# uber/aresdb

Hardware: AMD Instinct MI355X
Metric: rows/sec, 1B-row filter -> group-by-agg (whole job) (higher is better)
Workload: dtype u32 keys / f64 sums; 1 GPU; C3: filter d1<90 -> dims [floor(ts,3600), d1, d2, d3] (4 x uint32) -> SUM(m float32 -> float64) via HashReduce, validity bitmaps with 1% nulls, shard resident in HBM; rows_per_gpu=1000000000, batch_rows=67108864, batches=15, streams_per_query=2, parallelism=1 shard(s), one per GPU

## Files before the change

aresdb_amd/csrc/algo/hr_rtc_gen.hip:

```cpp
#include <cstdio>
#include <functional>
#include <sstream>
#include <string>
#include <vector>

#include "hr_kernels.hpp"
#include "hr_rtc_gen.hpp"

namespace ares {

namespace {

bool int_kind(int k) { return k == K_I32 || k == K_U32; }
bool col_kind(int k) { return k == K_I32 || k == K_U32 || k == K_F32; }

std::string hex(uint32_t v) {
  char b[16];
  snprintf(b, sizeof(b), "0x%08xu", v);
  return b;
}

std::string const_name(int slot) { return "a.k[" + std::to_string(slot) + "]"; }

bool gen_value(const RtcExpr &f, std::ostringstream &o, const char *v, const char *okb, const char *r, const std::string &kc,
// ... 692 lines not shown
         "  i0 = i0c;\n";
    for (int c = 0; c < nc; c++) {
      if (nullMask & (1u << c)) o << "  okc[" << c << "] = (r.win[" << c << "] >> ((i0c + a.bitOff[" << c << "]) & 7u)) & 0xFu;\n";
      else o << "  okc[" << c << "] = 0xFu;\n";
    }
    o << "#pragma unroll\n"
         "  for (int j = 0; j < 4; j++) {\n"
         "    u32 keep = ((u32)j >= sh && (int)(i0c + j) < a.length) ? 1u : 0u;\n";
    for (int k = 0; k < s.numFilters; k++) {
      const RtcExpr &e = s.filters[k];
      if (e.col < 0 || e.col >= nc) return "";
      o << "    {\n      const u32 v = r.v[" << e.col << "][j]; const u32 okb = (okc[" << e.col << "] >> j) & 1u;\n";
      if (!gen_compare(e, o, "v", "okb", "keep", const_name(const_slot_filter(k)))) return "";
      o << "    }\n";
    }
    o << "    alive[j] = keep;\n  }\n";
    for (int c = firstFilterCol; c < nc; c++) prefetch(c);
    if (constMeasure) {
      o << "  cv[0] = cv[1] = cv[2] = cv[3] = " << const_name(const_slot_measure()) << ";\n";
    } else {
      const RtcExpr &e = s.measure;
      if (e.col != nd) return "";
      o << "#pragma unroll\n  for (int j = 0; j < 4; j++) {\n"
           "    const u32 v = r.v[" << nd << "][j]; const u32 okb = (okc[" << nd << "] >> j) & 1u; u32 x;\n";
      if (!gen_value(e, o, "v", "okb", "x", const_name(const_slot_measure()), sort64)) return "";
      if (avg) {
        const int rk = e.rk;
        if (!(rk == K_F32 || rk == K_I32 || rk == K_U32) || !(s.measureDtype == Float64 || s.measureDtype == Int64)) return "";
        const bool f64 = s.measureDtype == Float64;
        const char *cvt = rk == K_F32 ? (f64 ? "x" : "__float_as_uint((float)(i64)__uint_as_float(x))")
                          : rk == K_I32 ? (f64 ? "__float_as_uint((float)(double)(i32)x)" : "__float_as_uint((float)(i64)(i32)x)")
                                        : (f64 ? "__float_as_uint((float)(double)x)" : "__float_as_uint((float)(i64)x)");
        o << "    cv[j] = okb ? " << cvt << " : 0u;\n"
             "    alive[j] |= (alive[j] & (okb ^ 1u)) << 31;\n";
      } else if (s.measureWidth == 8) {
        if (s.identity != 0) return "";
        o << "    cv[j] = okb ? x : 0u;\n";
      } else {
        const int target = s.measureDtype == Int32 ? K_I32 : s.measureDtype == Uint32 ? K_U32 : K_F32;
        if (!plain_store(e.rk, target)) return "";
        o << "    cv[j] = okb ? x : " << hex(static_cast<uint32_t>(s.identity)) << ";\n";
      }
      o << "  }\n";
      prefetch(nd);
    }
    if (SL.all4 && !sort64) {
    o << "  u32 h[4] = {0u, 0u, 0u, 0u}, okbytes[4] = {0u, 0u, 0u, 0u};\n";
    for (int d = 0; d < nd; d++) {
      const RtcExpr &e = s.dims[d];
      if (e.col != d || !plain_store(e.rk, e.outKind)) return "";
      o << "#pragma unroll\n  for (int j = 0; j < 4; j++) {\n"
           "    const u32 v = r.v[" << d << "][j]; const u32 okb = (okc[" << d << "] >> j) & 1u; u32 x;\n";
      if (!gen_value(e, o, "v", "okb", "x", const_name(const_slot_dim(d)))) return "";
      o << "    h[j] = mix(h[j], x); okbytes[j] |= okb << " << 8 * d << ";\n  }\n";
      prefetch(d);
    }
    o << "#pragma unroll\n  for (int j = 0; j < 4; j++) {\n    u32 g = h[j];\n";
    if (nd == 4) o << "    g = mix(g, okbytes[j]);\n";
    else o << "    { u32 k = okbytes[j] * 0xcc9e2d51u; k = rotl(k, 15) * 0x1b873593u; g ^= k; }\n";
    o << "    g ^= " << 5 * nd << "u; g ^= g >> 16; g *= 0x85ebca6bu; g ^= g >> 13; g *= 0xc2b2ae35u; g ^= g >> 16;\n"
         "    hh[j] = g;\n  }\n}\n";
    } else {
      for (int d = 0; d < nd; d++) o << "  u32 xv" << d << "[4], xo" << d << "[4];\n";
      for (int d = 0; d < nd; d++) {
        const RtcExpr &e = s.dims[d];
        if (e.col != d || !plain_store(e.rk, e.outKind) || (SL.width[d] != 4 && !int_kind(e.rk))) return "";
        o << "#pragma unroll\n  for (int j = 0; j < 4; j++) {\n"
             "    const u32 v = r.v[" << d << "][j]; const u32 okb = (okc[" << d << "] >> j) & 1u; u32 x;\n";
        if (!gen_value(e, o, "v", "okb", "x", const_name(const_slot_dim(d)))) return "";
        o << "    xv" << d << "[j] = x" << width_mask(SL.width[d]) << "; xo" << d << "[j] = okb;\n  }\n";
        prefetch(d);
      }
      o << "#pragma unroll\n  for (int j = 0; j < 4; j++) {\n";
      if (sort64) {
        o << "    u64 h64;\n";
        gen_row_hash64(o, SL, [](int d, int) { return "xv" + std::to_string(d) + "[j]"; }, [](int d) { return "xo" + std::to_string(d) + "[j]"; },
                       "h64", "    ");
        o << "    hh[j] = (u32)(h64 >> 32); cw[j] = (u32)h64;\n";
      } else {
        gen_row_hash(o, SL, [](int d) { return "xv" + std::to_string(d) + "[j]"; }, [](int d) { return "xo" + std::to_string(d) + "[j]"; },
                     "hh[j]", "    ");
      }
      o << "  }\n}\n";
    }
  }
  if (kind == RTC_SCAN_TABLE) {
    if (!gen_widen(o, s) || !gen_agg(o, s)) return "";
    kernel_body_table(o);
  } else if (kind == RTC_SCAN_COMPACT) {
    kernel_body_compact(o, s);
  } else {
    Lines16 rec{sort64 ? "cw[j]" : "0u"};
    if (avg) rec.row = "(a.rowBase + i0 + j) | (alive[j] & 0x80000000u)";
    kernel_body_lines16(o, s, rec);
  }
  return o.str();
}

std::string generate_vector(const RtcSpec &s) {
  const int nd = s.nd, vw = s.vectorVW, partBits = s.partBits;
  const bool hll = s.kind == RTC_HLL_SCAN, sort64 = hll || s.kind == RTC_SORT_VECTOR_SCAN;
  if (nd < 1 || nd > (sort64 ? kFusedDims : kGenericFusedDims) || (vw != 4 && vw != 8) || (sort64 && vw != 4)) return "";
  if (hll && (partBits < 1 || partBits > 9)) return "";
  const SlotLayout SL = slot_layout(s.dimWidth, nd, sort64 ? 16 : 4);
  if (!SL.ok || (!sort64 && !SL.all4)) return "";
  const int *width = SL.width;
  int wb[kFusedDims] = {};
  bool narrow = false, wide = false;
  int nw = 0;
  for (int d = 0; d < nd; d++) {
    narrow = narrow || width[d] != 4;
    wide = wide || width[d] > 4;
    wb[d] = nw;
    nw += width[d] > 4 ? width[d] / 4 : 1;
  }
  if (wide && SL.valueBytes > kSortVectorValueBytes) return "";
  std::ostringstream o;
  const int mq = vw / 4;
  o << kPrelude << (sort64 ? kPrelude64 : "") << args_text()
    << "#define ND " << nd << "\n#define MQ " << mq << "\n#define PB " << partBits << "\n#define NP " << (1 << partBits) << "\n";
  if (wide) o << "#define NW " << nw << "\nstruct Raw { u32 v[NW][4]; u32 ok[ND]; u32 m[MQ * 4]; };\n";
  else o << "struct Raw { u32 v[ND][4]; u32 ok[ND]; u32 m[MQ * 4]; };\n";
  o << "__device__ __forceinline__ void load_full(Raw &r, const Args &a, u32 i0) {\n";
  if (narrow) {
    for (int d = 0; d < nd; d++) {
      const int v = wb[d];
      if (width[d] > 4) {
        const int q = width[d] / 4;
        o << "  {\n    const PU32x4 *p = reinterpret_cast<const PU32x4 *>(reinterpret_cast<const u8 *>(a.vals[" << d << "]) + " << width[d] << "ull * i0);\n";
        for (int k = 0; k < q; k++) o << "    const PU32x4 t" << k << " = p[" << k << "];\n";
        o << "   ";
        for (int k = 0; k < q; k++)
          for (int e = 0; e < 4; e++) o << " r.v[" << v + (4 * k + e) % q << "][" << (4 * k + e) / q << "] = t" << k << ".v[" << e << "];";
        o << "\n  }\n";
      } else if (width[d] == 4)
        o << "  { const PU32x4 t = *reinterpret_cast<const PU32x4 *>(a.vals[" << d << "] + i0); r.v[" << v << "][0] = t.v[0]; r.v[" << v
          << "][1] = t.v[1]; r.v[" << v << "][2] = t.v[2]; r.v[" << v << "][3] = t.v[3]; }\n";
      else if (width[d] == 2)
        o << "  { const PU32x2 t = *reinterpret_cast<const PU32x2 *>(reinterpret_cast<const u8 *>(a.vals[" << d << "]) + 2ull * i0); r.v[" << v
          << "][0] = t.v[0] & 0xFFFFu; r.v[" << v << "][1] = t.v[0] >> 16; r.v[" << v << "][2] = t.v[1] & 0xFFFFu; r.v[" << v << "][3] = t.v[1] >> 16; }\n";
      else
        o << "  { const u32 t = reinterpret_cast<const PU32 *>(reinterpret_cast<const u8 *>(a.vals[" << d << "]) + i0)->v; r.v[" << v
          << "][0] = t & 0xFFu; r.v[" << v << "][1] = (t >> 8) & 0xFFu; r.v[" << v << "][2] = (t >> 16) & 0xFFu; r.v[" << v << "][3] = t >> 24; }\n";
      o << "  r.ok[" << d << "] = reinterpret_cast<const PU32 *>(a.nulls[" << d << "] + i0)->v;\n";
    }
  } else {
  o << "#pragma unroll\n"
       "  for (int d = 0; d < ND; d++) {\n"
       "    const PU32x4 t = *reinterpret_cast<const PU32x4 *>(a.vals[d] + i0);\n"
       "    r.v[d][0] = t.v[0]; r.v[d][1] = t.v[1]; r.v[d][2] = t.v[2]; r.v[d][3] = t.v[3];\n"
       "    r.ok[d] = reinterpret_cast<const PU32 *>(a.nulls[d] + i0)->v;\n"
       "  }\n";
  }
  o << ""
       "#pragma unroll\n"
       "  for (int q = 0; q < MQ; q++) {\n"
       "    const PU32x4 t = *reinterpret_cast<const PU32x4 *>(a.vals[ND] + (u64)i0 * MQ + 4 * q);\n"
       "    r.m[4 * q] = t.v[0]; r.m[4 * q + 1] = t.v[1]; r.m[4 * q + 2] = t.v[2]; r.m[4 * q + 3] = t.v[3];\n"
       "  }\n"
       "}\n"
       "__device__ __forceinline__ void load_tail(Raw &r, const Args &a, u32 i0) {\n";
  if (narrow) {
    for (int d = 0; d < nd; d++) {
      const char *elem = width[d] == 4 ? "a.vals[%d][i0 + j]" : width[d] == 2 ? "(u32)reinterpret_cast<const u16 *>(a.vals[%d])[i0 + j]" : "(u32)reinterpret_cast<const u8 *>(a.vals[%d])[i0 + j]";
      char buf[128];
      snprintf(buf, sizeof(buf), elem, d);
      o << "  r.ok[" << d << "] = 0u;\n"
           "  for (int j = 0; j < 4; j++) {\n"
           "    const bool in = (int)(i0 + j) < a.length;\n";
      if (width[d] > 4)
        for (int k = 0; k < width[d] / 4; k++)
          o << "    r.v[" << wb[d] + k << "][j] = in ? a.vals[" << d << "][" << width[d] / 4 << "ull * (i0 + j) + " << k << "] : 0u;\n";
      else
        o << "    r.v[" << wb[d] << "][j] = in ? " << buf << " : 0u;\n";
      o << "    r.ok[" << d << "] |= in ? (u32)a.nulls[" << d << "][i0 + j] << (8 * j) : 0u;\n"
           "  }\n";
    }
  } else {
  o << "#pragma unroll\n"
       "  for (int d = 0; d < ND; d++) {\n"
       "    r.ok[d] = 0u;\n"
       "    for (int j = 0; j < 4; j++) {\n"
       "      const bool in = (int)(i0 + j) < a.length;\n"
       "      r.v[d][j] = in ? a.vals[d][i0 + j] : 0u;\n"
       "      r.ok[d] |= in ? (u32)a.nulls[d][i0 + j] << (8 * j) : 0u;\n"
       "    }\n"
       "  }\n";
  }
  o << "  for (int j = 0; j < 4; j++)\n"
       "    for (int q = 0; q < MQ; q++) r.m[j * MQ + q] = (int)(i0 + j) < a.length ? a.vals[ND][(u64)(i0 + j) * MQ + q] : 0u;\n"
       "}\n"
       "__device__ __forceinline__ void eval4(const Raw &r, const Args &a, u32 i0, u32 (&hh)[4], u32 (&cv)[4], u32 (&cw)[4], u32 (&alive)[4]) {\n"
       "#pragma unroll\n"
       "  for (int j = 0; j < 4; j++) {\n"
       "    alive[j] = (int)(i0 + j) < a.length ? 1u : 0u;\n";
  if (sort64) {
    o << "    u64 h64;\n";
    gen_row_hash64(o, SL, [&](int d, int k) { return "r.v[" + std::to_string(wb[d] + k) + "][j]"; },
                   [](int d) { return "((r.ok[" + std::to_string(d) + "] >> (8 * j)) & 0xFFu)"; }, "h64", "    ");
    if (hll) o << "    h64 = (h64 & 0xFFFFFFFFFFFF0000ull) | (u64)(r.m[j] & 0x3FFFu);\n";
    o << "    hh[j] = (u32)(h64 >> 32);\n"
         "    cv[j] = r.m[j];\n"
         "    cw[j] = (u32)h64;\n"
         "  }\n"
         "}\n";
  } else {
  o << "    u32 h = 0u, okbytes = 0u;\n"
       "#pragma unroll\n"
       "    for (int d = 0; d < ND; d++) { h = mix(h, r.v[d][j]); okbytes |= ((r.ok[d] >> (8 * j)) & 0xFFu) << (8 * d); }\n";
  if (nd == 4) o << "    h = mix(h, okbytes);\n";
  else o << "    { u32 k = okbytes * 0xcc9e2d51u; k = rotl(k, 15) * 0x1b873593u; h ^= k; }\n";
  o << "    h ^= " << 5 * nd << "u; h ^= h >> 16; h *= 0x85ebca6bu; h ^= h >> 13; h *= 0xc2b2ae35u; h ^= h >> 16;\n"
       "    hh[j] = h;\n"
       "    cv[j] = r.m[j * MQ];\n"
       "    cw[j] = MQ == 2 ? r.m[j * MQ + MQ - 1] : 0u;\n"
       "  }\n"
       "}\n";
  }
  o << "__device__ __forceinline__ void load_tile(Raw &r, const Args &a, u32 i0) { if ((int)(i0 + 3u) < a.length) load_full(r, a, i0); else if ((int)i0 < a.length) load_tail(r, a, i0); }\n"
       "__device__ __forceinline__ void eval4p(Raw &r, const Args &a, u32 &i0, u32 (&hh)[4], u32 (&cv)[4], u32 (&cw)[4], u32 (&alive)[4], u32 i0n) {\n"
       "  eval4(r, a, i0, hh, cv, cw, alive);\n"
       "  load_tile(r, a, i0n);\n"
       "}\n";
  Lines16 rec{"cw[j]"};
  if (hll)
    rec.part = "(((hh[j] ^ (cw[j] * 0x9E3779B1u)) * 0x85EBCA6Bu) >> (32 - PB))";
  else if (sort64)
    rec.part = "(a.pad ? (((hh[j] >> a.chunkTiles) ^ ((((hh[j] >> a.chunkTiles) >> PB) * 0x9E3779B1u) >> 23)) & (NP - 1u)) "
               ": (PB ? hh[j] >> (32 - (PB ? PB : 1)) : 0u))";
  kernel_body_lines16(o, s, rec);
  return o.str();
}

std::string generate_merge(const RtcSpec &s) {
  const int nd = s.nd, partBits = s.partBits, image = s.image, vectorVW = s.kind == RTC_VECTOR_MERGE ? s.vectorVW : 0;
  const bool compact = s.compact != 0, regionA = s.regionA != 0;
  if (nd < 1 || nd > kFusedDims) return "";
  if (image && vectorVW) return "";
  if (compact && (vectorVW || partBits < 3)) return "";
  if (partBits < 2) return "";
  const SlotLayout SL = slot_layout(s.dimWidth, nd, 4);
  if (!SL.ok || (vectorVW && !SL.all4)) return "";
  std::ostringstream o;
  o << kPrelude
    << "struct MArgs { const u32 *vals[" << kFusedCols << "]; const u8 *nulls[" << kFusedCols << "]; const u32 *recB; const u32 *countsB;\n"
       "  const u32 *prevRanges; const u8 *prevDims; const u8 *prevValues; u8 *dimOut; u8 *outValues; u32 *outCount; u32 *outRanges;\n"
       "  u64 prevCapacity, outCapacity; u32 bitOff[" << kFusedCols << "]; u32 capB, streams, prevSize, chunkRows; u64 *phases; u32 k[" << kNumConsts << "]; u32 pad;\n"
       "  const uint4 *recA; const u32 *cursorsA; u64 capA;\n"
       "  const uint4 *imgIn; uint4 *imgOut; const u32 *imgInCount; u32 *imgOutCount; u32 *hostOut; u32 knownOut, pad2; };\n"
       "#define FINISH() { __syncthreads(); if (threadIdx.x == 0u && a.hostOut) { __threadfence(); \\\n"
       "  if (atomicAdd(a.outCount + 4, 1u) == gridDim.x - 1u) { __threadfence(); const volatile u32 *oc = a.outCount; \\\n"
       "    a.hostOut[0] = oc[0]; a.hostOut[1] = oc[1]; a.hostOut[2] = oc[2]; a.hostOut[3] = oc[3]; } } }\n"
       "#define ND " << nd << "\n#define VB " << SL.valueBytes << "\n#define PB " << partBits << "\n#define NP " << (1 << partBits) << "\n"
       "#define SLOTS " << hr::kSlots << "\n#define LIMIT " << hr::kMergeLimit << "u\n#define RANGEWORDS " << hr::kRangeWords
    << "\n#define MAXRANGES " << hr::kMaxRanges << "u\n"
       "#define HMASK ((1u << (32 - PB)) - 1u)\n#define OCC 0x40000000u\n#define NEWG 0x80000000u\n";
  gen_widen(o, s);
  if (!gen_agg(o, s)) return "";
  if (s.phases)
    o << "#define STAMP(k) if (threadIdx.x == 0u) a.phases[(u64)blockIdx.x * 8u + (k)] = __builtin_amdgcn_s_memrealtime();\n";
  else
    o << "#define STAMP(k)\n";
  o << "#define BUCKETS (SLOTS / 4)\n"
       "struct Probe { u32 b, slot; bool done, isNew; };\n"
       "__device__ __forceinline__ void probe_round(u32 *sKeys, u32 *sClaimed, u32 *sOverflow, Probe &q, u32 want, u32 claimKey) {\n"
       "  const uint4 k = *reinterpret_cast<const uint4 *>(sKeys + 4u * q.b);\n"
       "  const bool e0 = k.x == 0u, e1 = k.y == 0u, e2 = k.z == 0u, e3 = k.w == 0u;\n"
       "  const bool m0 = (k.x & ~NEWG) == want, m1 = (k.y & ~NEWG) == want, m2 = (k.z & ~NEWG) == want, m3 = (k.w & ~NEWG) == want;\n"
       "  const bool anyM = m0 | m1 | m2 | m3, anyE = e0 | e1 | e2 | e3;\n"
       "  const u32 mi = m0 ? 0u : m1 ? 1u : m2 ? 2u : 3u, ei = e0 ? 0u : e1 ? 1u : e2 ? 2u : 3u;\n"
       "  const u32 mk = m0 ? k.x : m1 ? k.y : m2 ? k.z : k.w;\n"
       "  const bool active = !q.done, hit = active & anyM;\n"
       "  q.slot = hit ? 4u * q.b + mi : q.slot;\n"
       "  q.isNew = hit ? (mk & NEWG) != 0u : q.isNew;\n"
       "  bool claimed = false;\n"
       "  if (active & !anyM & anyE) {\n"
       "    u32 expected = 0u;\n"
       "    if (__hip_atomic_compare_exchange_strong(sKeys + 4u * q.b + ei, &expected, claimKey, __ATOMIC_RELAXED, __ATOMIC_RELAXED, __HIP_MEMORY_SCOPE_WORKGROUP)) {\n"
       "      if (__hip_atomic_fetch_add(sClaimed, 1u, __ATOMIC_RELAXED, __HIP_MEMORY_SCOPE_WORKGROUP) >= LIMIT)\n"
       "        __hip_atomic_store(sOverflow, 1u, __ATOMIC_RELAXED, __HIP_MEMORY_SCOPE_WORKGROUP);\n"
       "      q.slot = 4u * q.b + ei; q.isNew = true; claimed = true;\n"
       "    }\n"
       "  }\n"
       "  q.b = (active & !anyM & !anyE) ? (q.b + 1u) & (BUCKETS - 1u) : q.b;\n"
       "  q.done = q.done | hit | claimed;\n"
       "}\n"
       "__device__ __forceinline__ void insert(u32 *sKeys, u32 *sRows, u64 *sVals, u32 *sClaimed, u32 *sOverflow, u32 row, u32 h, u64 value, bool batch) {\n"
       "  const u32 want = (h & HMASK) | OCC;\n"
       "  Probe q; q.b = h & (BUCKETS - 1u); q.slot = 0u; q.done = false; q.isNew = false;\n"
       "  for (u32 tries = 0u; tries < 4u * BUCKETS && !q.done; tries++) probe_round(sKeys, sClaimed, sOverflow, q, want, batch ? want | NEWG : want);\n"
       "  if (q.done) {\n"
       "    if (q.isNew || !batch) __hip_atomic_fetch_min(sRows + q.slot, row, __ATOMIC_RELAXED, __HIP_MEMORY_SCOPE_WORKGROUP);\n"
       "    agg(sVals + q.slot, value);\n"
       "  } else {\n"
       "    __hip_atomic_store(sOverflow, 1u, __ATOMIC_RELAXED, __HIP_MEMORY_SCOPE_WORKGROUP);\n"
       "  }\n"
       "}\n";
  if (vectorVW == 8)
    o << "#define QCAP 96u\n#define QW 4u\n#define QDRAIN 32u\n#define VALB(z, w) ((((u64)(w)) << 32) | (z))\n";
  else if (vectorVW == 4)
    o << "#define QCAP 128u\n#define QW 3u\n#define QDRAIN 64u\n#define VALB(z, w) ((u64)(z))\n";
  else
    o << "#define QCAP 128u\n#define QW 3u\n#define QDRAIN 64u\n#define VALB(z, w) widen(z)\n";
  o << "struct Seg { const uint4 *ptr; u32 n, rem, rb; };\n"
       "struct Stage { uint4 r[4]; u32 n[4], rem[4], rb[4]; };\n"
       "__device__ __forceinline__ void drain(u32 *queue, u32 first, u32 count, u32 lane, u32 *sKeys, u32 *sRows, u64 *sVals, u32 *sClaimed, u32 *sOverflow) {\n"
       "  asm volatile(\"s_waitcnt lgkmcnt(0)\" ::: \"memory\");\n"
       "  if (lane < count) {\n"
       "    const u32 e = QW * (first + lane);\n"
       "    const u32 row = queue[e], h = queue[e + 1u], z = queue[e + 2u], w = QW == 4u ? queue[e + QW - 1u] : 0u;\n"
       "    insert(sKeys, sRows, sVals, sClaimed, sOverflow, row, h, VALB(z, w), true);\n"
       "  }\n"
       "  asm volatile(\"s_waitcnt lgkmcnt(0)\" ::: \"memory\");\n"
       "}\n"
       "__device__ __forceinline__ void consume_one(bool valid, u32 row, u32 h, u32 z, u32 w, u32 lane, u32 *sKeys, u32 *sRows, u64 *sVals, u32 *sClaimed, u32 *sOverflow, u32 *queue, u32 &qn) {\n"
       "  const u32 b = h & (BUCKETS - 1u), want = (h & HMASK) | OCC;\n"
       "  const uint4 k = *reinterpret_cast<const uint4 *>(sKeys + 4u * b);\n"
       "  const bool m0 = (k.x & ~NEWG) == want, m1 = (k.y & ~NEWG) == want, m2 = (k.z & ~NEWG) == want, m3 = (k.w & ~NEWG) == want;\n"
       "  const bool hit = valid && (m0 || m1 || m2 || m3);\n"
       "  if (hit) {\n"
       "    const u32 mi = m0 ? 0u : m1 ? 1u : m2 ? 2u : 3u;\n"
       "    const u32 mk = m0 ? k.x : m1 ? k.y : m2 ? k.z : k.w;\n"
       "    if (mk & NEWG) __hip_atomic_fetch_min(sRows + 4u * b + mi, row, __ATOMIC_RELAXED, __HIP_MEMORY_SCOPE_WORKGROUP);\n"
       "    agg(sVals + 4u * b + mi, VALB(z, w));\n"
       "  }\n"
       "  const bool pend = valid && !hit;\n"
       "  const u64 m = __ballot(pend);\n"
       "  if (m) {\n"
       "    if (pend) {\n"
       "      const u32 e = QW * (qn + __builtin_amdgcn_mbcnt_hi((u32)(m >> 32), __builtin_amdgcn_mbcnt_lo((u32)m, 0u)));\n"
       "      queue[e] = row; queue[e + 1u] = h; queue[e + 2u] = z;\n"
       "      if (QW == 4u) queue[e + QW - 1u] = w;\n"
       "    }\n"
       "    qn += (u32)__popcll(m);\n"
       "    if (qn >= QDRAIN) { const u32 take = qn < 64u ? qn : 64u; qn -= take; drain(queue, qn, take, lane, sKeys, sRows, sVals, sClaimed, sOverflow); }\n"
       "  }\n"
       "}\n";
  if (compact)
    o << "__device__ __forceinline__ void consume(const Stage &s, u32 lane, u32 p, u32 *sKeys, u32 *sRows, u64 *sVals, u32 *sClaimed, u32 *sOverflow, u32 *queue, u32 &qn) {\n"
         "  const u32 pos = 2u * (lane & 3u);\n"
         "  const u32 recBase = (lane >> 3) * 14u + 7u * ((lane >> 2) & 1u);\n"
         "#pragma unroll\n"
         "  for (int k = 0; k < 4; k++) {\n"
         "    const u64 hdr = ((u64)(u32)__builtin_amdgcn_mov_dpp((int)s.r[k].y, 0x00, 0xF, 0xF, true) << 32) | (u32)__builtin_amdgcn_mov_dpp((int)s.r[k].x, 0x00, 0xF, 0xF, true);\n"
         "#pragma unroll\n"
         "    for (u32 j = 0u; j < 2u; j++) {\n"
         "      const u32 ph = pos + j;\n"
         "      const u32 k7 = ph ? ph - 1u : 0u;\n"
         "      const bool valid = lane < s.n[k] && ph != 0u && recBase + k7 < s.rem[k];\n"
         "      const u32 z = j ? s.r[k].z : s.r[k].x, hw = j ? s.r[k].w : s.r[k].y;\n"
         "      const u32 lo9 = (u32)(hdr >> (9u * k7)) & 511u;\n"
         "      const u32 h = (p << (32 - PB)) | (hw >> PB);\n"
         "      const u32 row = s.rb[k] + (((hw & ((1u << PB) - 1u)) << 9) | lo9);\n"
         "      consume_one(valid, row, h, z, 0u, lane, sKeys, sRows, sVals, sClaimed, sOverflow, queue, qn);\n"
         "    }\n"
         "  }\n"
         "}\n";
  else
    o << "__device__ __forceinline__ void consume(const Stage &s, u32 lane, u32 p, u32 *sKeys, u32 *sRows, u64 *sVals, u32 *sClaimed, u32 *sOverflow, u32 *queue, u32 &qn) {\n"
         "#pragma unroll\n"
         "  for (int k = 0; k < 4; k++) {\n"
         "    const bool valid = lane < s.n[k] && s.r[k].x != 0xFFFFFFFFu;\n"
         "    consume_one(valid, s.r[k].x, s.r[k].y, s.r[k].z, s.r[k].w, lane, sKeys, sRows, sVals, sClaimed, sOverflow, queue, qn);\n"
         "  }\n"
         "}\n";
  if (!vectorVW) o << "__device__ __forceinline__ void eval_row(const MArgs &a, u32 row, u32 (&bits)[ND], u32 (&ok)[ND]) {\n";
  for (int d = 0; d < nd && !vectorVW; d++) {
    const RtcExpr &e = s.dims[d];
    const int c = e.col;
    if (c < 0 || c >= kFusedCols || !plain_store(e.rk, e.outKind) || (SL.width[d] != 4 && !int_kind(e.rk))) return "";
    o << "  {\n    const u32 v = " << column_elem(s.step[c], e.akind == K_I32, "a.vals[" + std::to_string(c) + "]", "row") << ";\n";
    if (s.nullMask & (1u << c)) o << "    const u32 bit = row + a.bitOff[" << c << "]; const u32 okb = (a.nulls[" << c << "][bit >> 3] >> (bit & 7u)) & 1u;\n";
    else o << "    const u32 okb = 1u;\n";
    o << "    u32 x;\n";
    if (!gen_value(e, o, "v", "okb", "x", const_name(const_slot_dim(d)))) return "";
    o << "    bits[" << d << "] = x; ok[" << d << "] = okb;\n  }\n";
  }
  if (!vectorVW) o << "}\n";
  const bool wide = s.aggWidth == 8;
  o << "extern \"C\" __global__ void __launch_bounds__(1024) hr_merge_rtc(MArgs a) {\n"
       "  __shared__ __attribute__((aligned(16))) u32 sKeys[SLOTS];\n"
       "  __shared__ __attribute__((aligned(16))) u32 sRows[SLOTS];\n"
       "  __shared__ __attribute__((aligned(16))) u64 sVals[SLOTS];\n"
       "  __shared__ u32 sRunCount[256];\n"
       "  __shared__ u32 sQueue[16u * QCAP * QW];\n"
       "  __shared__ u32 sClaimed, sOverflow, sCount, sBase, sEmit;\n"
       "  const u32 tid = threadIdx.x, lane = tid & 63u, wave = tid >> 6, p = blockIdx.x;\n"
       "  STAMP(0)\n";
  if (image == 2)
    o << "  {\n"
         "    const uint4 *img = a.imgIn + (u64)p * SLOTS;\n"
         "    for (u32 i = tid; i < SLOTS / 4u; i += 1024u) {\n"
         "      reinterpret_cast<uint4 *>(sKeys)[i] = img[i];\n"
         "      reinterpret_cast<uint4 *>(sRows)[i] = img[SLOTS / 4u + i];\n"
         "    }\n"
         "    for (u32 i = tid; i < SLOTS / 2u; i += 1024u) reinterpret_cast<uint4 *>(sVals)[i] = img[SLOTS / 2u + i];\n"
         "    if (tid == 0u) { sClaimed = a.imgInCount[p]; sOverflow = 0u; sCount = 0u; sEmit = 0u; }\n"
         "  }\n";
  else
    o << "  for (u32 s = tid; s < SLOTS; s += 1024u) { sKeys[s] = 0u; sRows[s] = 0xFFFFFFFFu; sVals[s] = IDENT; }\n"
         "  if (tid == 0u) { sClaimed = 0u; sOverflow = 0u; sCount = 0u; sEmit = 0u; }\n";
  o << "  const u32 G = a.streams;\n"
       "  if (tid < G) sRunCount[tid] = a.countsB[(u64)tid * NP + p];\n"
       "  const u32 *ranges = a.prevRanges ? a.prevRanges + (u64)p * RANGEWORDS : nullptr;\n"
       "  u32 nRanges = ranges ? ranges[0] : 0u;\n"
       "  if (nRanges > MAXRANGES) { if (tid == 0u) a.outCount[2] = 1u; nRanges = 0u; }\n"
       "  __syncthreads();\n"
       "  STAMP(1)\n"
       "  {\n"
       "    const u8 *nullsIn = a.prevDims + (u64)VB * a.prevCapacity;\n"
       "    for (u32 r = 0u; r < nRanges; r++) {\n"
       "      const u32 start = ranges[1u + 2u * r], cnt = ranges[2u + 2u * r];\n"
       "      for (u32 i0 = 0u; i0 < cnt; i0 += 4096u) {\n"
       "        u32 hh[4], rr[4]; u64 vv[4]; bool okk[4];\n"
       "#pragma unroll\n"
       "        for (int k = 0; k < 4; k++) {\n"
       "          const u32 i = i0 + (u32)k * 1024u + tid;\n"
       "          okk[k] = i < cnt;\n"
       "          const u32 row = start + (okk[k] ? i : 0u);\n"
       "          rr[k] = row;\n"
       "          okk[k] = okk[k] && row < a.prevSize;\n"
       "          const u32 safe = row < a.prevSize ? row : 0u;\n"
       "          u32 h = 0u;\n";
  if (SL.all4) {
    o << "          u32 okbytes = 0u;\n"
         "#pragma unroll\n"
         "          for (int d = 0; d < ND; d++) {\n"
         "            h = mix(h, *reinterpret_cast<const u32 *>(a.prevDims + (u64)(4 * d) * a.prevCapacity + 4ull * safe));\n"
         "            okbytes |= (u32)nullsIn[(u64)d * a.prevCapacity + safe] << (8 * d);\n"
         "          }\n";
    if (nd == 4) o << "          h = mix(h, okbytes);\n";
    else o << "          { u32 kk = okbytes * 0xcc9e2d51u; kk = rotl(kk, 15) * 0x1b873593u; h ^= kk; }\n";
    o << "          h ^= " << 5 * nd << "u; h ^= h >> 16; h *= 0x85ebca6bu; h ^= h >> 13; h *= 0xc2b2ae35u; h ^= h >> 16;\n";
  } else {
    for (int d = 0; d < nd; d++)
      o << "          const u32 pv" << d << " = " << slot_load(SL, d, "a.prevDims", "a.prevCapacity", "safe") << ", po" << d
        << " = (u32)nullsIn[(u64)" << d << " * a.prevCapacity + safe];\n";
    gen_row_hash(o, SL, [](int d) { return "pv" + std::to_string(d); }, [](int d) { return "po" + std::to_string(d); }, "h", "          ");
  }
  o <<
       "          hh[k] = h;\n"
    << (wide ? "          vv[k] = reinterpret_cast<const u64 *>(a.prevValues)[safe];\n"
             : "          vv[k] = reinterpret_cast<const u32 *>(a.prevValues)[safe];\n")
    << "        }\n"
       "#pragma unroll\n"
       "        for (int k = 0; k < 4; k++) {\n"
       "          const u32 i = i0 + (u32)k * 1024u + tid;\n"
       "          if (i >= cnt) continue;\n"
       "          if (!okk[k] || (PB && (hh[k] >> (32 - (PB ? PB : 1))) != p)) { a.outCount[2] = 1u; continue; }\n"
       "          insert(sKeys, sRows, sVals, &sClaimed, &sOverflow, rr[k], hh[k], vv[k], false);\n"
       "        }\n"
       "      }\n"
       "    }\n"
       "  }\n"
       "  __syncthreads();\n"
       "  STAMP(2)\n";
  if (regionA)
    o << "  {\n"
         "    const u32 cur = a.cursorsA[p];\n"
         "    const u32 nA = cur < a.capA ? cur : (u32)a.capA;\n"
         "    const uint4 *recs = a.recA + (u64)p * a.capA;\n"
         "    for (u32 i = tid; i < nA; i += 1024u) {\n"
         "      const uint4 r = recs[i];\n"
         "      insert(sKeys, sRows, sVals, &sClaimed, &sOverflow, r.x, r.y, ((u64)r.w << 32) | r.z, true);\n"
         "    }\n"
         "  }\n"
         "  __syncthreads();\n";
  o << "  u32 maxRun = 0u;\n"
       "  for (u32 g = lane; g < G; g += 64u) { const u32 c = sRunCount[g]; maxRun = c > maxRun ? c : maxRun; }\n"
       "#pragma unroll\n"
       "  for (int off = 32; off > 0; off >>= 1) { const u32 t = (u32)__shfl_xor((int)maxRun, off); maxRun = t > maxRun ? t : maxRun; }\n"
       "  const u32 LPR = (maxRun + " << (compact ? "13u) / 14u" : "7u) / 8u") << ";\n"
       "  if (G > 0u && LPR <= 4u && LPR <= a.capB" << (compact ? "" : " / 8u") << ") {\n"
       "    u32 qn = 0u;\n"
       "    u32 *queue = sQueue + wave * (QCAP * QW);\n"
       "    const u32 units = G * 8u * LPR;\n"
       "    for (u32 base = 0u; base < units; base += 4096u) {\n"
       "      Stage s;\n"
       "#pragma unroll\n"
       "      for (int k = 0; k < 4; k++) {\n"
       "        const u32 u = base + (u32)k * 1024u + tid;\n"
       "        const bool in = u < units;\n"
       "        const u32 ul = in ? u >> 3 : 0u, g = ul / LPR, l = ul - g * LPR, cnt = in ? sRunCount[g] : 0u;\n"
    << (compact ? "        const u32 here = cnt > l * 14u ? cnt - l * 14u : 0u;\n"
                  "        s.r[k] = reinterpret_cast<const uint4 *>(a.recB)[(((u64)g * NP + p) * a.capB + l) * 8u + (u & 7u)];\n"
                  "        s.n[k] = here ? 64u : 0u; s.rem[k] = (lane >> 3) * 14u + here; s.rb[k] = a.prevSize + g * a.chunkRows;\n"
                : "        const u32 here = cnt > l * 8u ? cnt - l * 8u : 0u;\n"
                  "        s.r[k] = reinterpret_cast<const uint4 *>(a.recB)[((u64)g * NP + p) * a.capB + l * 8u + (u & 7u)];\n"
                  "        s.n[k] = (u & 7u) < here ? 64u : 0u; s.rem[k] = 0u; s.rb[k] = 0u;\n")
    << "      }\n"
       "      consume(s, lane, p, sKeys, sRows, sVals, &sClaimed, &sOverflow, queue, qn);\n"
       "    }\n"
       "    while (qn) { const u32 take = qn < 64u ? qn : 64u; qn -= take; drain(queue, qn, take, lane, sKeys, sRows, sVals, &sClaimed, &sOverflow); }\n"
       "  } else\n"
       "  if (G > 0u) {\n"
       "    const uint4 *dummy = reinterpret_cast<const uint4 *>(a.recB);\n"
       "    u32 j = 0u, off = 0u, qn = 0u;\n"
       "    u32 *queue = sQueue + wave * (QCAP * QW);\n"
       "    const u32 myRuns = (G + 15u - wave) / 16u;\n"
       "    const u32 myCnt = lane < myRuns ? sRunCount[wave + 16u * lane] : 0u;\n";
  if (compact)
    o << "    auto next = [&]() -> Seg {\n"
         "      Seg c{dummy, 0u, 0u, 0u};\n"
         "      while (j < myRuns) {\n"
         "        const u32 cnt = (u32)__builtin_amdgcn_readlane((int)myCnt, (int)j);\n"
         "        const u32 units = ((cnt + 13u) / 14u) * 8u;\n"
         "        if (off < units) {\n"
         "          c.ptr = reinterpret_cast<const uint4 *>(a.recB) + ((u64)(wave + 16u * j) * NP + p) * a.capB * 8u + off;\n"
         "          c.n = units - off < 64u ? units - off : 64u;\n"
         "          c.rem = cnt - (off >> 3) * 14u;\n"
         "          c.rb = a.prevSize + (wave + 16u * j) * a.chunkRows;\n"
         "          off += 64u;\n"
         "          break;\n"
         "        }\n"
         "        j++; off = 0u;\n"
         "      }\n"
         "      return c;\n"
         "    };\n";
  else
    o << "    auto next = [&]() -> Seg {\n"
         "      Seg c{dummy, 0u, 0u, 0u};\n"
         "      while (j < myRuns) {\n"
         "        const u32 cnt = (u32)__builtin_amdgcn_readlane((int)myCnt, (int)j);\n"
         "        if (off < cnt) {\n"
         "          c.ptr = reinterpret_cast<const uint4 *>(a.recB) + ((u64)(wave + 16u * j) * NP + p) * a.capB + off;\n"
         "          c.n = cnt - off < 64u ? cnt - off : 64u;\n"
         "          off += 64u;\n"
         "          break;\n"
         "        }\n"
         "        j++; off = 0u;\n"
         "      }\n"
         "      return c;\n"
         "    };\n";
  o << "    auto load = [&](Stage &s) {\n"
       "#pragma unroll\n"
       "      for (int k = 0; k < 4; k++) {\n"
       "        const Seg c = next();\n"
       "        s.n[k] = c.n; s.rem[k] = c.rem; s.rb[k] = c.rb;\n"
       "        s.r[k] = c.ptr[lane < c.n ? lane : (c.n ? c.n - 1u : 0u)];\n"
       "      }\n"
       "    };\n"
       "    Stage s0, s1, s2;\n"
       "    load(s0);\n"
       "    load(s1);\n"
       "    for (;;) {\n"
       "      load(s2);\n"
       "      if (!s0.n[0]) break;\n"
       "      consume(s0, lane, p, sKeys, sRows, sVals, &sClaimed, &sOverflow, queue, qn);\n"
       "      load(s0);\n"
       "      if (!s1.n[0]) break;\n"
       "      consume(s1, lane, p, sKeys, sRows, sVals, &sClaimed, &sOverflow, queue, qn);\n"
       "      load(s1);\n"
       "      if (!s2.n[0]) break;\n"
       "      consume(s2, lane, p, sKeys, sRows, sVals, &sClaimed, &sOverflow, queue, qn);\n"
       "    }\n"
       "    while (qn) { const u32 take = qn < 64u ? qn : 64u; qn -= take; drain(queue, qn, take, lane, sKeys, sRows, sVals, &sClaimed, &sOverflow); }\n"
       "  }\n"
       "  __syncthreads();\n"
       "  STAMP(3)\n"
       "  if (sOverflow) { if (tid == 0u) a.outCount[3] = 1u; FINISH() return; }\n";
  const char *kStoreKeysPos =
      "    for (u32 i = tid; i < SLOTS / 4u; i += 1024u) {\n"
      "      img[i] = reinterpret_cast<const uint4 *>(sKeys)[i];\n"
      "      img[SLOTS / 4u + i] = reinterpret_cast<const uint4 *>(sRows)[i];\n"
      "    }\n";
  const char *kStoreVals = "    for (u32 i = tid; i < SLOTS / 2u; i += 1024u) img[SLOTS / 2u + i] = reinterpret_cast<const uint4 *>(sVals)[i];\n";
  if (image == 2) {
    o << "  u32 mineNew = 0u;\n"
         "#pragma unroll\n"
         "  for (int k = 0; k < SLOTS / 1024; k++) mineNew += (sKeys[tid + (u32)k * 1024u] & NEWG) != 0u;\n"
         "  if (mineNew) __hip_atomic_fetch_add(&sCount, mineNew, __ATOMIC_RELAXED, __HIP_MEMORY_SCOPE_WORKGROUP);\n"
         "  __syncthreads();\n"
         "  const u32 totalNew = sCount;\n"
         "  if (tid == 0u) sBase = a.prevSize + (totalNew ? atomicAdd(a.outCount, totalNew) : 0u);\n"
         "  __syncthreads();\n"
         "  STAMP(4)\n"
         "  u8 *nullsOut = a.dimOut + (u64)VB * a.outCapacity;\n"
         "  if (totalNew) {\n"
         "#pragma unroll\n"
         "    for (int half = 0; half < 2; half++) {\n"
         "      u32 dv[4][ND], nv[4][ND], at[4]; bool has[4];\n"
         "#pragma unroll\n"
         "      for (int kk = 0; kk < 4; kk++) {\n"
         "        const u32 s = tid + (u32)(half * 4 + kk) * 1024u;\n"
         "        has[kk] = (sKeys[s] & NEWG) != 0u;\n"
         "        const u64 m = __ballot(has[kk]);\n"
         "        u32 waveBase = 0u;\n"
         "        if (lane == 0u && m) waveBase = __hip_atomic_fetch_add(&sEmit, (u32)__popcll(m), __ATOMIC_RELAXED, __HIP_MEMORY_SCOPE_WORKGROUP);\n"
         "        waveBase = (u32)__builtin_amdgcn_readfirstlane((int)waveBase);\n"
         "        at[kk] = sBase + waveBase + __builtin_amdgcn_mbcnt_hi((u32)(m >> 32), __builtin_amdgcn_mbcnt_lo((u32)m, 0u));\n"
         "        if (has[kk]) eval_row(a, sRows[s] - a.prevSize, dv[kk], nv[kk]);\n"
         "      }\n"
         "#pragma unroll\n"
         "      for (int kk = 0; kk < 4; kk++) {\n"
         "        if (!has[kk]) continue;\n"
         "        const u32 s = tid + (u32)(half * 4 + kk) * 1024u;\n";
    for (int d = 0; d < nd; d++)
      o << "        " << slot_store(SL, d, "a.dimOut", "a.outCapacity", "at[kk]", "dv[kk][" + std::to_string(d) + "]") << " nullsOut[(u64)" << d
        << " * a.outCapacity + at[kk]] = (u8)nv[kk][" << d << "];\n";
    o << "        sRows[s] = at[kk];\n"
         "        sKeys[s] &= ~NEWG;\n"
         "      }\n"
         "    }\n"
         "  }\n"
         "  __syncthreads();\n"
         "  {\n"
         "    uint4 *img = a.imgOut + (u64)p * SLOTS;\n"
         "    const u32 newCount = a.imgInCount[p] + totalNew;\n"
         "    if (a.imgOutCount[p] != newCount) {\n"
      << kStoreKeysPos
      << "    }\n"
      << kStoreVals
      << "    __syncthreads();\n"
         "    if (tid == 0u) a.imgOutCount[p] = newCount;\n"
         "  }\n"
         "  if (a.knownOut < a.prevSize) {\n"
         "    const u8 *nullsIn = a.prevDims + (u64)VB * a.prevCapacity;\n"
         "    const u32 n = a.prevSize - a.knownOut, share = (n + NP - 1u) / NP;\n"
         "    const u32 lo = a.knownOut + p * share, hi = lo + share < a.prevSize ? lo + share : a.prevSize;\n"
         "    for (u32 r = lo + tid; r < hi; r += 1024u) {\n";
    for (int d = 0; d < nd; d++)
      o << "      " << slot_store(SL, d, "a.dimOut", "a.outCapacity", "r", slot_load(SL, d, "a.prevDims", "a.prevCapacity", "r")) << " nullsOut[(u64)" << d
        << " * a.outCapacity + r] = nullsIn[(u64)" << d << " * a.prevCapacity + r];\n";
    o << "    }\n"
         "  }\n"
         "  STAMP(5)\n"
         "  FINISH()\n"
         "}\n";
    return o.str();
  }
  o <<
       "  u32 mineCount = 0u;\n"
       "#pragma unroll\n"
       "  for (int k = 0; k < SLOTS / 1024; k++) mineCount += sKeys[tid + (u32)k * 1024u] != 0u;\n"
       "  if (mineCount) __hip_atomic_fetch_add(&sCount, mineCount, __ATOMIC_RELAXED, __HIP_MEMORY_SCOPE_WORKGROUP);\n"
       "  __syncthreads();\n"
       "  const u32 total = sCount;\n"
       "  if (tid == 0u) {\n"
       "    u32 base = 0u;\n"
       "    if (total) base = atomicAdd(a.outCount, total);\n"
       "    sBase = base;\n"
       "    if (a.outRanges) { u32 *o = a.outRanges + (u64)p * RANGEWORDS; o[0] = total ? 1u : 0u; o[1] = base; o[2] = total; }\n"
       "  }\n"
       "  __syncthreads();\n"
       "  STAMP(4)\n"
    << (image == 1 ? "" : "  if (!total) { FINISH() return; }\n")
    << "  const u8 *nullsIn = a.prevDims + (u64)VB * a.prevCapacity;\n"
       "  u8 *nullsOut = a.dimOut + (u64)VB * a.outCapacity;\n"
       "#pragma unroll\n"
       "  for (int half = 0; half < 2; half++) {\n"
       "    u32 dv[4][ND], nv[4][ND], at[4]; bool has[4];\n"
       "#pragma unroll\n"
       "    for (int kk = 0; kk < 4; kk++) {\n"
       "      const u32 s = tid + (u32)(half * 4 + kk) * 1024u;\n"
       "      has[kk] = sKeys[s] != 0u;\n"
       "      const u64 m = __ballot(has[kk]);\n"
       "      u32 waveBase = 0u;\n"
       "      if (lane == 0u && m) waveBase = __hip_atomic_fetch_add(&sEmit, (u32)__popcll(m), __ATOMIC_RELAXED, __HIP_MEMORY_SCOPE_WORKGROUP);\n"
       "      waveBase = (u32)__builtin_amdgcn_readfirstlane((int)waveBase);\n"
       "      at[kk] = sBase + waveBase + __builtin_amdgcn_mbcnt_hi((u32)(m >> 32), __builtin_amdgcn_mbcnt_lo((u32)m, 0u));\n"
       "      if (!has[kk]) continue;\n"
       "      const u32 row = sRows[s];\n"
    << (vectorVW ? "" : "      if (row >= a.prevSize) { eval_row(a, row - a.prevSize, dv[kk], nv[kk]); continue; }\n");
  if (SL.all4) {
    o << "#pragma unroll\n"
         "      for (int d = 0; d < ND; d++) {\n"
         "        dv[kk][d] = *reinterpret_cast<const u32 *>(a.prevDims + (u64)(4 * d) * a.prevCapacity + 4ull * row);\n"
         "        nv[kk][d] = nullsIn[(u64)d * a.prevCapacity + row];\n"
         "      }\n";
  } else {
    for (int d = 0; d < nd; d++)
      o << "      dv[kk][" << d << "] = " << slot_load(SL, d, "a.prevDims", "a.prevCapacity", "row") << "; nv[kk][" << d << "] = nullsIn[(u64)" << d
        << " * a.prevCapacity + row];\n";
  }
  o << "    }\n"
       "#pragma unroll\n"
       "    for (int kk = 0; kk < 4; kk++) {\n"
       "      if (!has[kk]) continue;\n"
       "      const u32 s = tid + (u32)(half * 4 + kk) * 1024u;\n";
  if (SL.all4) {
    o << "#pragma unroll\n"
         "      for (int d = 0; d < ND; d++) {\n"
         "        *reinterpret_cast<u32 *>(a.dimOut + (u64)(4 * d) * a.outCapacity + 4ull * at[kk]) = dv[kk][d];\n"
         "        nullsOut[(u64)d * a.outCapacity + at[kk]] = (u8)nv[kk][d];\n"
         "      }\n";
  } else {
    for (int d = 0; d < nd; d++)
      o << "      " << slot_store(SL, d, "a.dimOut", "a.outCapacity", "at[kk]", "dv[kk][" + std::to_string(d) + "]") << " nullsOut[(u64)" << d
        << " * a.outCapacity + at[kk]] = (u8)nv[kk][" << d << "];\n";
  }
  o << (wide ? "      reinterpret_cast<u64 *>(a.outValues)[at[kk]] = sVals[s];\n"
             : "      reinterpret_cast<u32 *>(a.outValues)[at[kk]] = (u32)sVals[s];\n")
    << (image == 1 ? "      sRows[s] = at[kk];\n      sKeys[s] &= ~NEWG;\n" : "")
    << "    }\n"
       "  }\n";
  if (image == 1)
    o << "  __syncthreads();\n"
         "  {\n"
         "    uint4 *img = a.imgOut + (u64)p * SLOTS;\n"
      << kStoreKeysPos << kStoreVals
      << "    if (tid == 0u) a.imgOutCount[p] = total;\n"
         "  }\n";
  o <<
       "  STAMP(5)\n"
       "  FINISH()\n"
       "}\n";
  return o.str();
}

enum ExprRole { FILTER, DIMENSION, MEASURE };
RtcExpr spec_expr(const FusedExpr &e, ExprRole role) {
  RtcExpr x{};
  x.col = e.col; x.akind = e.f.akind; x.arity = e.f.arity; x.I = e.f.I;
  if (role != FILTER) x.rk = e.f.rk;
  if (role == DIMENSION) x.outKind = e.outKind;
  if (e.f.arity != 2) return x;
  x.functor = e.f.functor; x.bok = e.f.bok != 0;
  if (role == FILTER) return x;
  x.bkind = e.f.bkind; x.divLike = e.f.divLike != 0;
  if (x.divLike) x.bbits = e.f.bbits;
  return x;
}
RtcSpec spec_of(RtcKind kind, int nd, int partBits, bool stamps = true) {
  RtcSpec s{};
  s.kind = kind; s.nd = nd; s.partBits = partBits;
  s.phases = stamps && phases_enabled();
  return s;
}
void spec_column(RtcSpec &s, const FusedPlanD &plan, int c) {
  s.step[c] = fused_col_step(plan, c);
  if (plan.cols[c].nulls) s.nullMask |= 1u << c;
}
void spec_dims(RtcSpec &s, const FusedPlanD &plan) {
  for (int d = 0; d < s.nd && d < kFusedDims; d++) {
    s.dimWidth[d] = fused_dim_width(plan, d);
    s.dims[d] = spec_expr(plan.dims[d], DIMENSION);
  }
}
void spec_agg(RtcSpec &s, const AggSpec &a, const hr::Widen &w) {
  s.aggVtype = a.vtype; s.aggIdentity = a.identity;
  if (a.vtype == V_U32 || a.vtype == V_I32) s.aggOp = a.op;
  s.widenMode = w.mode;
  if (w.mode) { s.widenRk = w.rk; s.widenDtype = w.dtype; }
}
RtcSpec spec_plan_scan(RtcKind kind, const FusedPlanD &plan, int nd, int partBits) {
  RtcSpec s = spec_of(kind, nd, partBits, kind != RTC_SCAN_TABLE);
  s.numCols = plan.numCols; s.numFilters = plan.numFilters;
  for (int c = 0; c < plan.numCols && c < kFusedCols; c++) spec_column(s, plan, c);
  for (int k = 0; k < plan.numFilters && k < kFusedFilters; k++) s.filters[k] = spec_expr(plan.filters[k], FILTER);
  spec_dims(s, plan);
  s.measureAvg = plan.measureAvg != 0;
  s.constMeasure = plan.measure.col < 0;
  if (!s.constMeasure) {
    s.measure = spec_expr(plan.measure, MEASURE);
    s.measureWidth = plan.measureWidth; s.identity = plan.identity;
    if (s.measureAvg || plan.measureWidth != 8) s.measureDtype = plan.measureDtype;
  }
  return s;
}
RtcSpec spec_vector(RtcKind kind, int nd, const int *widths, int vw, int partBits) {
  RtcSpec s = spec_of(kind, nd, partBits);
  for (int d = 0; d < nd && d < kFusedDims; d++) s.dimWidth[d] = widths ? widths[d] : 4;
  s.vectorVW = vw;
  return s;
}

}

const char *rtc_entry_name(int32_t kind) {
  switch (kind) {
    case RTC_SCAN_SORT64: case RTC_SORT_VECTOR_SCAN: return "sr_scan_rtc";
    case RTC_HLL_SCAN: return "hll_scan_rtc";
    case RTC_MERGE: case RTC_VECTOR_MERGE: return "hr_merge_rtc";
    default: return "hr_scan_rtc";
  }
}

RtcSpec rtc_spec_scan(const FusedPlanD &plan, int nd, int partBits, bool compact) {
  return spec_plan_scan(compact ? RTC_SCAN_COMPACT : RTC_SCAN_LINES16, plan, nd, partBits);
}
RtcSpec rtc_spec_sort_scan(const FusedPlanD &plan, int nd, int partBits) { return spec_plan_scan(RTC_SCAN_SORT64, plan, nd, partBits); }
RtcSpec rtc_spec_table_scan(const FusedPlanD &plan, int nd, int partBits, const AggSpec &a, const hr::Widen &w) {
  RtcSpec s = spec_plan_scan(RTC_SCAN_TABLE, plan, nd, partBits);
  spec_agg(s, a, w);
  return s;
}
RtcSpec rtc_spec_vector_scan(int nd, int vw, int partBits) { return spec_vector(RTC_VECTOR_SCAN, nd, nullptr, vw, partBits); }
RtcSpec rtc_spec_sort_vector_scan(int nd, const int *widths, int partBits) { return spec_vector(RTC_SORT_VECTOR_SCAN, nd, widths, 4, partBits); }
RtcSpec rtc_spec_hll_scan(int nd, const int *widths, int partBits) { return spec_vector(RTC_HLL_SCAN, nd, widths, 4, partBits); }
RtcSpec rtc_spec_merge(const FusedPlanD &plan, int nd, int partBits, const AggSpec &a, const hr::Widen &w, bool compact, bool regionA,
                       int image) {
  RtcSpec s = spec_of(RTC_MERGE, nd, partBits);
  spec_dims(s, plan);
  for (int d = 0; d < nd && d < kFusedDims; d++)
    if (plan.dims[d].col >= 0 && plan.dims[d].col < kFusedCols) spec_column(s, plan, plan.dims[d].col);
  spec_agg(s, a, w);
  s.aggWidth = a.width;
  s.compact = compact; s.regionA = regionA; s.image = image;
  return s;
}
RtcSpec rtc_spec_vector_merge(int nd, int vw, int partBits, const AggSpec &a) {
  RtcSpec s = spec_vector(RTC_VECTOR_MERGE, nd, nullptr, vw, partBits);
  spec_agg(s, a, hr::Widen{0, 0, 0});
  s.aggWidth = a.width;
  return s;
}

std::string rtc_source(const RtcSpec &s) {
  switch (s.kind) {
    case RTC_SCAN_LINES16: case RTC_SCAN_COMPACT: case RTC_SCAN_TABLE: case RTC_SCAN_SORT64: return generate(s);
    case RTC_VECTOR_SCAN: case RTC_SORT_VECTOR_SCAN: case RTC_HLL_SCAN: return generate_vector(s);
    case RTC_MERGE: case RTC_VECTOR_MERGE: return generate_merge(s);
    default: return "";
  }
}

}
```

Before: 93.11 billion rows/s.

## Pack tail of one run and head of next into a single wave segment

The merge kernel's segment iterator now fills a 64-lane load with the tail of one run plus the head of the next run, instead of issuing a partially-filled segment per run tail. Segment metadata is packed into one word per stage (count, split point, remaining records, run offset), and consume becomes a template that picks per-lane row base and remaining count based on which side of the split the lane is in. The aim is to cut idle lanes and extra iterations when many runs are short. In exchange it adds per-lane selects and bit-packing limits, such as remaining counts clamped to 127 and a run-delta field limited to 4 bits.

```diff
diff --git a/aresdb_amd/csrc/algo/hr_rtc_gen.hip b/aresdb_amd/csrc/algo/hr_rtc_gen.hip
--- a/aresdb_amd/csrc/algo/hr_rtc_gen.hip
+++ b/aresdb_amd/csrc/algo/hr_rtc_gen.hip
@@ -1018,8 +1018,17 @@
     o << "#define QCAP 128u\n#define QW 3u\n#define QDRAIN 64u\n#define VALB(z, w) ((u64)(z))\n";
   else
     o << "#define QCAP 128u\n#define QW 3u\n#define QDRAIN 64u\n#define VALB(z, w) widen(z)\n";
-  o << "struct Seg { const uint4 *ptr; u32 n, rem, rb; };\n"
-       "struct Stage { uint4 r[4]; u32 n[4], rem[4], rb[4]; };\n"
+  o << "struct Seg { const uint4 *ptr, *ptrB; u32 m, rb; };\n"
+       "struct Stage { uint4 r[4]; u32 n[4], rem[4], rb[4];\n"
+       "  __device__ __forceinline__ void pick(int k, u32, u32, u32 &n_, u32 &rem_, u32 &rb_) const { n_ = n[k]; rem_ = rem[k]; rb_ = rb[k]; }\n"
+       "  __device__ __forceinline__ bool none(int) const { return false; } };\n"
+    << (compact ? "#define SEG_N(m) (((m) & 15u) << 3)\n#define SEG_T(m) ((((m) >> 4) & 15u) << 3)\n"
+                : "#define SEG_N(m) ((m) & 0xFFu)\n#define SEG_T(m) (((m) >> 8) & 0xFFu)\n")
+    << "struct PStage { uint4 r[4]; u32 m[4], rb[4];\n"
+       "  __device__ __forceinline__ void pick(int k, u32 lane, u32 stride, u32 &n_, u32 &rem_, u32 &rb_) const {\n"
+       "    const u32 mm = m[k]; const bool inA = lane < SEG_T(mm);\n"
+       "    n_ = SEG_N(mm); rem_ = inA ? (mm >> 8) & 127u : (mm >> 15) & 255u; rb_ = inA ? rb[k] : rb[k] + ((mm >> 23) & 15u) * stride; }\n"
+       "  __device__ __forceinline__ bool none(int k) const { return m[k] == 0u; } };\n"
        "__device__ __forceinline__ void drain(u32 *queue, u32 first, u32 count, u32 lane, u32 *sKeys, u32 *sRows, u64 *sVals, u32 *sClaimed, u32 *sOverflow) {\n"
        "  asm volatile(\"s_waitcnt lgkmcnt(0)\" ::: \"memory\");\n"
        "  if (lane < count) {\n"
@@ -1053,30 +1062,34 @@
        "  }\n"
        "}\n";
   if (compact)
-    o << "__device__ __forceinline__ void consume(const Stage &s, u32 lane, u32 p, u32 *sKeys, u32 *sRows, u64 *sVals, u32 *sClaimed, u32 *sOverflow, u32 *queue, u32 &qn) {\n"
+    o << "template <class S> __device__ __forceinline__ void consume(const S &s, u32 lane, u32 p, u32 stride, u32 *sKeys, u32 *sRows, u64 *sVals, u32 *sClaimed, u32 *sOverflow, u32 *queue, u32 &qn) {\n"
          "  const u32 pos = 2u * (lane & 3u);\n"
          "  const u32 recBase = (lane >> 3) * 14u + 7u * ((lane >> 2) & 1u);\n"
          "#pragma unroll\n"
          "  for (int k = 0; k < 4; k++) {\n"
+         "    if (s.none(k)) break;\n"
          "    const u64 hdr = ((u64)(u32)__builtin_amdgcn_mov_dpp((int)s.r[k].y, 0x00, 0xF, 0xF, true) << 32) | (u32)__builtin_amdgcn_mov_dpp((int)s.r[k].x, 0x00, 0xF, 0xF, true);\n"
+         "    u32 segN, segRem, segRb; s.pick(k, lane, stride, segN, segRem, segRb);\n"
          "#pragma unroll\n"
          "    for (u32 j = 0u; j < 2u; j++) {\n"
          "      const u32 ph = pos + j;\n"
          "      const u32 k7 = ph ? ph - 1u : 0u;\n"
-         "      const bool valid = lane < s.n[k] && ph != 0u && recBase + k7 < s.rem[k];\n"
+         "      const bool valid = lane < segN && ph != 0u && recBase + k7 < segRem;\n"
          "      const u32 z = j ? s.r[k].z : s.r[k].x, hw = j ? s.r[k].w : s.r[k].y;\n"
          "      const u32 lo9 = (u32)(hdr >> (9u * k7)) & 511u;\n"
          "      const u32 h = (p << (32 - PB)) | (hw >> PB);\n"
-         "      const u32 row = s.rb[k] + (((hw & ((1u << PB) - 1u)) << 9) | lo9);\n"
+         "      const u32 row = segRb + (((hw & ((1u << PB) - 1u)) << 9) | lo9);\n"
          "      consume_one(valid, row, h, z, 0u, lane, sKeys, sRows, sVals, sClaimed, sOverflow, queue, qn);\n"
          "    }\n"
          "  }\n"
          "}\n";
   else
-    o << "__device__ __forceinline__ void consume(const Stage &s, u32 lane, u32 p, u32 *sKeys, u32 *sRows, u64 *sVals, u32 *sClaimed, u32 *sOverflow, u32 *queue, u32 &qn) {\n"
+    o << "template <class S> __device__ __forceinline__ void consume(const S &s, u32 lane, u32 p, u32 stride, u32 *sKeys, u32 *sRows, u64 *sVals, u32 *sClaimed, u32 *sOverflow, u32 *queue, u32 &qn) {\n"
          "#pragma unroll\n"
          "  for (int k = 0; k < 4; k++) {\n"
-         "    const bool valid = lane < s.n[k] && s.r[k].x != 0xFFFFFFFFu;\n"
+         "    if (s.none(k)) break;\n"
+         "    u32 segN, segRem, segRb; s.pick(k, lane, stride, segN, segRem, segRb);\n"
+         "    const bool valid = lane < segN && s.r[k].x != 0xFFFFFFFFu;\n"
          "    consume_one(valid, s.r[k].x, s.r[k].y, s.r[k].z, s.r[k].w, lane, sKeys, sRows, sVals, sClaimed, sOverflow, queue, qn);\n"
          "  }\n"
          "}\n";
@@ -1205,7 +1218,7 @@
                   "        s.r[k] = reinterpret_cast<const uint4 *>(a.recB)[((u64)g * NP + p) * a.capB + l * 8u + (u & 7u)];\n"
                   "        s.n[k] = (u & 7u) < here ? 64u : 0u; s.rem[k] = 0u; s.rb[k] = 0u;\n")
     << "      }\n"
-       "      consume(s, lane, p, sKeys, sRows, sVals, &sClaimed, &sOverflow, queue, qn);\n"
+       "      consume(s, lane, p, 0u, sKeys, sRows, sVals, &sClaimed, &sOverflow, queue, qn);\n"
        "    }\n"
        "    while (qn) { const u32 take = qn < 64u ? qn : 64u; qn -= take; drain(queue, qn, take, lane, sKeys, sRows, sVals, &sClaimed, &sOverflow); }\n"
        "  } else\n"
@@ -1213,62 +1226,74 @@
        "    const uint4 *dummy = reinterpret_cast<const uint4 *>(a.recB);\n"
        "    u32 j = 0u, off = 0u, qn = 0u;\n"
        "    u32 *queue = sQueue + wave * (QCAP * QW);\n"
-       "    const u32 myRuns = (G + 15u - wave) / 16u;\n"
-       "    const u32 myCnt = lane < myRuns ? sRunCount[wave + 16u * lane] : 0u;\n";
-  if (compact)
-    o << "    auto next = [&]() -> Seg {\n"
-         "      Seg c{dummy, 0u, 0u, 0u};\n"
-         "      while (j < myRuns) {\n"
-         "        const u32 cnt = (u32)__builtin_amdgcn_readlane((int)myCnt, (int)j);\n"
-         "        const u32 units = ((cnt + 13u) / 14u) * 8u;\n"
-         "        if (off < units) {\n"
-         "          c.ptr = reinterpret_cast<const uint4 *>(a.recB) + ((u64)(wave + 16u * j) * NP + p) * a.capB * 8u + off;\n"
-         "          c.n = units - off < 64u ? units - off : 64u;\n"
-         "          c.rem = cnt - (off >> 3) * 14u;\n"
-         "          c.rb = a.prevSize + (wave + 16u * j) * a.chunkRows;\n"
-         "          off += 64u;\n"
-         "          break;\n"
-         "        }\n"
-         "        j++; off = 0u;\n"
-         "      }\n"
-         "      return c;\n"
-         "    };\n";
-  else
-    o << "    auto next = [&]() -> Seg {\n"
-         "      Seg c{dummy, 0u, 0u, 0u};\n"
-         "      while (j < myRuns) {\n"
-         "        const u32 cnt = (u32)__builtin_amdgcn_readlane((int)myCnt, (int)j);\n"
-         "        if (off < cnt) {\n"
-         "          c.ptr = reinterpret_cast<const uint4 *>(a.recB) + ((u64)(wave + 16u * j) * NP + p) * a.capB + off;\n"
-         "          c.n = cnt - off < 64u ? cnt - off : 64u;\n"
-         "          off += 64u;\n"
-         "          break;\n"
-         "        }\n"
-         "        j++; off = 0u;\n"
-         "      }\n"
-         "      return c;\n"
-         "    };\n";
-  o << "    auto load = [&](Stage &s) {\n"
+       "    const u32 wv = (u32)__builtin_amdgcn_readfirstlane((int)wave);\n"
+       "    const u32 myRuns = (G + 15u - wv) / 16u;\n"
+       "    const u32 myCnt = lane < myRuns ? sRunCount[wv + 16u * lane] : 0u;\n";
+  o << "    u32 units = 0u, rem = 0u;\n"
+       "    const uint4 *base = dummy;\n"
+       "    auto open = [&]() {\n"
+       "      units = 0u; off = 0u;\n"
+       "      while (j < myRuns) {\n"
+       "        rem = (u32)__builtin_amdgcn_readlane((int)myCnt, (int)j);\n"
+       "        if (rem) break;\n"
+       "        j++;\n"
+       "      }\n"
+       "      if (j >= myRuns) return;\n"
+    << (compact ? "      units = ((rem + 13u) / 14u) * 8u;\n"
+                  "      base = reinterpret_cast<const uint4 *>(a.recB) + ((u64)(wv + 16u * j) * NP + p) * a.capB * 8u;\n"
+                : "      units = rem;\n"
+                  "      base = reinterpret_cast<const uint4 *>(a.recB) + ((u64)(wv + 16u * j) * NP + p) * a.capB;\n")
+    << "    };\n"
+       "    open();\n"
+       "    auto next = [&]() -> Seg {\n"
+       "      Seg c{dummy, dummy, 0u, 0u};\n"
+       "      if (off >= units) {\n"
+       "        if (!units) return c;\n"
+       "        j++; open();\n"
+       "        if (!units) return c;\n"
+       "      }\n"
+       "      const u32 left = units - off;\n"
+       "      c.ptr = base + off;\n"
+    << (compact ? "      c.m = (rem < 127u ? rem : 127u) << 8; c.rb = a.prevSize + (wv + 16u * j) * a.chunkRows;\n"
+                  "      if (left >= 64u) { c.m |= 8u | (8u << 4); off += 64u; rem -= 112u; return c; }\n"
+                : "      if (left >= 64u) { c.m = 64u | (64u << 8); off += 64u; return c; }\n")
+    << "      u32 n = left;\n"
+       "      const u32 jA = j;\n"
+       "      j++; open();\n"
+       "      if (units) {\n"
+       "        off = units < 64u - left ? units : 64u - left;\n"
+       "        n = left + off;\n"
+       "        c.ptrB = base;\n"
+    << (compact ? "        c.m |= (((rem < 127u ? rem : 127u) + (left >> 3) * 14u) << 15) | ((j - jA) << 23);\n"
+                  "        rem -= (off >> 3) * 14u;\n" : "")
+    << "      }\n"
+    << (compact ? "      c.m |= (n >> 3) | ((left >> 3) << 4);\n" : "      c.m = n | (left << 8);\n")
+    << "      return c;\n"
+       "    };\n";
+  o << "    auto load = [&](PStage &s) {\n"
        "#pragma unroll\n"
        "      for (int k = 0; k < 4; k++) {\n"
        "        const Seg c = next();\n"
-       "        s.n[k] = c.n; s.rem[k] = c.rem; s.rb[k] = c.rb;\n"
-       "        s.r[k] = c.ptr[lane < c.n ? lane : (c.n ? c.n - 1u : 0u)];\n"
+       "        s.m[k] = c.m; s.rb[k] = c.rb;\n"
+       "        const u32 n = SEG_N(c.m), t = SEG_T(c.m);\n"
+       "        const u32 l = lane < n ? lane : (n ? n - 1u : 0u);\n"
+       "        const uint4 *q = l < t ? c.ptr + l : c.ptrB + (l - t);\n"
+       "        s.r[k] = *q;\n"
        "      }\n"
        "    };\n"
-       "    Stage s0, s1, s2;\n"
+       "    PStage s0, s1, s2;\n"
        "    load(s0);\n"
        "    load(s1);\n"
        "    for (;;) {\n"
        "      load(s2);\n"
-       "      if (!s0.n[0]) break;\n"
-       "      consume(s0, lane, p, sKeys, sRows, sVals, &sClaimed, &sOverflow, queue, qn);\n"
+       "      if (!s0.m[0]) break;\n"
+       "      consume(s0, lane, p, 16u * a.chunkRows, sKeys, sRows, sVals, &sClaimed, &sOverflow, queue, qn);\n"
        "      load(s0);\n"
-       "      if (!s1.n[0]) break;\n"
-       "      consume(s1, lane, p, sKeys, sRows, sVals, &sClaimed, &sOverflow, queue, qn);\n"
+       "      if (!s1.m[0]) break;\n"
+       "      consume(s1, lane, p, 16u * a.chunkRows, sKeys, sRows, sVals, &sClaimed, &sOverflow, queue, qn);\n"
        "      load(s1);\n"
-       "      if (!s2.n[0]) break;\n"
-       "      consume(s2, lane, p, sKeys, sRows, sVals, &sClaimed, &sOverflow, queue, qn);\n"
+       "      if (!s2.m[0]) break;\n"
+       "      consume(s2, lane, p, 16u * a.chunkRows, sKeys, sRows, sVals, &sClaimed, &sOverflow, queue, qn);\n"
        "    }\n"
        "    while (qn) { const u32 take = qn < 64u ? qn : 64u; qn -= take; drain(queue, qn, take, lane, sKeys, sRows, sVals, &sClaimed, &sOverflow); }\n"
        "  }\n"
```

Measured after the change: 93.07 billion rows/s. Within noise of the previous version (-0.1%).
